# mazpie/genrl

Measured on AMD Instinct MI355X. Metric: world-model+imag update steps/sec (B32xL32x64x64x3), higher is better.
Workload: dtype f32 (storage, accumulation, every non-GEMM kernel and the fp32-MFMA GEMMs; the forward / dgrad / weight-gradient products of the imagination rollout, of the Dense+LN+SiLU chains from 192 rows up and of the encoder / decoder convolutions take fp32 operands pre-split into two fp16 planes of the scaled

## Files before the change

genrl_amd/csrc/gemm_planes.hip:

```cpp
#include "common.h"
#include "genrl_hip.h"
#include <type_traits>

typedef __bf16 bf16x8_t __attribute__((ext_vector_type(8)));
typedef _Float16 f16x8_t __attribute__((ext_vector_type(8)));
typedef unsigned u32x4 __attribute__((ext_vector_type(4)));

namespace {

struct PlaneSeg {
  const u16* a; long a_ld, a_plane;
  const u16* b; long b_ld, b_plane;
  int k;
  const float* a_inv; const float* b_inv;
};

struct SampleEpi {
  const float* q;
  long ldq;
  float* sample; long lds;
  u16* sp; long sld, splane; float* sinv;
  float a;
};

struct ConvGather {
  int H, W, C, k, Ho, Wo, K;
  int s;
  int sHo, sWo, sCo;
};

__device__ __host__ __forceinline__ long ln_slab(int tn) { return (long)(tn - 1) * 65536; }
struct LnEpi {
  const float* gamma; const float* beta;
  float eps; int act;
  float* y; long ldy;
  u16* yp; long yld, yplane; float* yinv;
  float* mean; float* rstd;
  float* part;
  unsigned* sync;
};

struct PairSel {
  const u16* b; long b_ld, b_plane; const float* b_inv;
  float* C; long ldc; int N, accumulate;
  int tn0, nx;
};

__device__ __forceinline__ float pow2_ratio(float a, float b) {
  const int ea = (int)((__builtin_bit_cast(unsigned, a) >> 23) & 255u), eb = (int)((__builtin_bit_cast(unsigned, b) >> 23) & 255u);
  const int e = min(max(ea - eb + 127, 1), 254);
  return __builtin_bit_cast(float, (unsigned)e << 23);
}
__device__ __forceinline__ bool zero_row_inv(float inv) { return __builtin_bit_cast(unsigned, inv) == (4u << 23); }

__device__ __forceinline__ void glds16(const void* g, unsigned lds_byte_addr) {
  __builtin_amdgcn_global_load_lds((const __attribute__((address_space(1))) void*)g,
                                   (__attribute__((address_space(3))) void*)(uintptr_t)lds_byte_addr, 16, 0, 0);
}

template <int N> __device__ __forceinline__ void wait_vm() { asm volatile("s_waitcnt vmcnt(%0)" ::"i"(N) : "memory"); }

template <int TM, int TN, int BK, int NACC, int FMT, int NS, bool FOLD, bool CONV, int PF, bool LNE, bool IS_PAIR>
__device__ __forceinline__ void gemm_planes_body(PlaneSeg s0, PlaneSeg s1, float* __restrict__ C, long ldc,
                                                 const float* __restrict__ bias, int M, int N, int accumulate,
                                                 int tiles_m, int tiles_n, int xcd_m, SampleEpi smp, ConvGather cg, LnEpi ln, PairSel pr) {
  static_assert(!LNE || (TM * TN == 1 && FMT == 1 && !CONV && PF == 0), "LayerNorm epilogue: 64x64 h2 tile");
  static_assert(!IS_PAIR || (TM * TN == 1 && FMT == 1 && !CONV && PF == 0 && !LNE), "pair of products: 64x64 h2 tile");
  constexpr int BM = 64 * TM, BN = 64 * TN;
  static_assert(!(FMT == 1 && FOLD) || (BM == 64 && BN == 64), "segment fold: 64x64 h2 tile");
  constexpr int NPL = FMT ? 2 : 3, NPROD = FMT ? 3 : 6;
  constexpr int ROWB = BK * 2;
  constexpr int CPR = ROWB / 16;
  constexpr int RPC = 1024 / ROWB;
  constexpr int A_BYTES = NPL * BM * ROWB, B_BYTES = NPL * BN * ROWB, STAGE = A_BYTES + B_BYTES;
  constexpr int APIECES = A_BYTES / 1024, BPIECES = B_BYTES / 1024;
  static_assert(APIECES % 2 == 0 && BPIECES % 2 == 0, "pieces split over two waves per operand");
  constexpr int NPA = APIECES / 2, NPB = BPIECES / 2;
  constexpr int NPMAX = NPA > NPB ? NPA : NPB;
  constexpr int KS = BK / 16;
  static_assert(PF == 0 || (BK == 64 && !CONV), "prefetch: 128-byte tile rows, plain operands");
  constexpr int NPF = PF ? TM : 0;
  constexpr int EPI = FMT == 1 ? 4 * (BM + 2 * BN) : 0, EPI_AT = NS * STAGE + (PF ? 1024 : 0);
  constexpr int LN_AT = EPI_AT + EPI, LN_G = LN_AT, LN_B = LN_AT + 4096, LN_R = LN_AT + 8192, LN_U = LN_AT + 9216, LN_T = LN_AT + 9472, LN_BYTES = LNE ? 9728 : 0;
  __shared__ __attribute__((aligned(1024))) unsigned char lds[EPI_AT + EPI + LN_BYTES];
// ... 1276 lines not shown
};
struct SplitBatch {
  int n;
  int blk0[33];
  SplitEntry e[32];
};
__device__ __forceinline__ int batch_entry(const SplitBatch& b, int blk) {
  int i = 0;
  while (i + 1 < b.n && blk >= b.blk0[i + 1]) ++i;
  return i;
}
__global__ __launch_bounds__(256) void split_h2_rows_batch_kernel(SplitBatch b) {
  const int i = batch_entry(b, blockIdx.x);
  const SplitEntry& e = b.e[i];
  const int row = (blockIdx.x - b.blk0[i]) * 4 + (threadIdx.x >> 6), lane = threadIdx.x & 63;
  if (row >= e.R) return;
  const float* xr = e.src + (long)row * e.ldx;
  float m = 0.f;
  for (int c = lane; c < e.Cn; c += 64) m = fmaxf(m, fabsf(xr[c]));
  const float iv = h2_inv_of(wave_max(m)), sc = h2_scale_of(iv);
  if (lane == 0) e.inv[row] = iv;
  u16* o = e.out + (long)row * e.ld_out;
  for (int c = 2 * lane; c < e.ld_out; c += 128) {
    unsigned h, l;
    h2_split2(c < e.Cn ? xr[c] * sc : 0.f, c + 1 < e.Cn ? xr[c + 1] * sc : 0.f, h, l);
    *reinterpret_cast<unsigned*>(o + c) = h;
    *reinterpret_cast<unsigned*>(o + e.plane + c) = l;
  }
}
__global__ __launch_bounds__(256) void h2_colmax_batch_kernel(SplitBatch b) {
  __shared__ float part[8][32];
  const int i = batch_entry(b, blockIdx.x);
  const SplitEntry& e = b.e[i];
  const int tx = threadIdx.x & 31, ty = threadIdx.x >> 5;
  const int c = (blockIdx.x - b.blk0[i]) * 32 + tx;
  float m = 0.f;
  if (c < e.Cn) {
    int r = ty;
    for (; r + 56 < e.R; r += 64) {
      float v[8];
#pragma unroll
      for (int u = 0; u < 8; ++u) v[u] = e.src[(long)(r + 8 * u) * e.ldx + c];
#pragma unroll
      for (int u = 0; u < 8; ++u) m = fmaxf(m, fabsf(v[u]));
    }
    for (; r < e.R; r += 8) m = fmaxf(m, fabsf(e.src[(long)r * e.ldx + c]));
  }
  part[ty][tx] = m;
  __syncthreads();
  if (ty == 0 && c < e.Cn) {
#pragma unroll
    for (int k = 1; k < 8; ++k) m = fmaxf(m, part[k][tx]);
    e.inv[c] = h2_inv_of(m);
  }
}
__global__ __launch_bounds__(256) void split_h2_t_batch_kernel(SplitBatch b) {
  __shared__ float tile[32][33];
  const int i = batch_entry(b, blockIdx.x);
  const SplitEntry& e = b.e[i];
  const int tiles_x = (int)((e.ld_out + 31) / 32);
  const int t = blockIdx.x - b.blk0[i];
  const int tx = threadIdx.x & 31, ty = threadIdx.x >> 5;
  const int ro = (t / tiles_x) * 32, co = (t % tiles_x) * 32;
#pragma unroll
  for (int k = 0; k < 4; ++k) {
    const int a = ty + 8 * k;
    const int r = co + a, c = ro + tx;
    tile[tx][a] = (r < e.R && c < e.Cn) ? e.src[(long)r * e.ldx + c] : 0.f;
  }
  __syncthreads();
#pragma unroll
  for (int k = 0; k < 4; ++k) {
    const int a = ty + 8 * k;
    const int r = ro + a, c = co + tx;
    if (r < e.Cn && c < e.ld_out) {
      unsigned h, l;
      h2_split2(c < e.R ? tile[a][tx] * h2_scale_of(e.inv[r]) : 0.f, 0.f, h, l);
      u16* o = e.out + (long)r * e.ld_out + c;
      o[0] = (u16)(h & 0xFFFFu); o[e.plane] = (u16)(l & 0xFFFFu);
    }
  }
}

static inline void log_launch(const char* family, long M, long N, long K, double bytes) { genrl_log_launch(family, M, N, K, bytes); }
static inline double kk_bytes(long M, long N, long K) { return 4.0 * ((double)M * K + (double)N * K + (double)M * N); }
static bool use_wide(int N) {
  static const int mode = getenv("GENRL_HL_WIDE") ? atoi(getenv("GENRL_HL_WIDE")) : 1;
  if (mode == 0) return false;
  const int c128 = cdiv(N, 128) * 128, c192 = cdiv(N, 192) * 192;
  return c192 < c128 || (mode == 2 && c192 == c128);
}
static bool use_tall96(int N, int K) {
  return N <= 96 && K >= 1024;
}
static bool hl_on() { static const bool on = !getenv("GENRL_PLANES_HL") || getenv("GENRL_PLANES_HL")[0] != '0'; return on; }
int g_planes_force_tile = 0;

}

unsigned g_planes_route = 0;
int g_planes_route_splits = 0;
static inline void route_reset() { g_planes_route = 0; g_planes_route_splits = 0; }
static inline void route(unsigned bit) { g_planes_route |= bit; }

extern "C" {

void genrl_log_launch(const char* family, long M, long N, long K, double operand_bytes) {
  static FILE* f = getenv("GENRL_GEMM_LOG") ? fopen(getenv("GENRL_GEMM_LOG"), "w") : nullptr;
  if (f) { fprintf(f, "%s %ld %ld %ld %.0f\n", family, M, N, K, operand_bytes); fflush(f); }
}

int genrl_planes_force_tile(int t) { const int p = g_planes_force_tile; g_planes_force_tile = t; return p; }
long genrl_planes_last_route(void) { return (long)g_planes_route | ((long)g_planes_route_splits << 32); }

int genrl_split_x3(const float* x, long ldx, int R, int Cn, uint16_t* out, long ld_out, long plane, int transpose,
                   void* stream) {
  GENRL_ENTER();
  const int Ro = transpose ? Cn : R, Co = transpose ? R : Cn;
  if (R <= 0 || Cn <= 0 || ld_out < Co) return GENRL_EINVAL;
  dim3 grid(cdiv(ld_out, 32), cdiv(Ro, 32));
  split_x3_kernel<<<grid, 256, 0, (hipStream_t)stream>>>(x, ldx, R, Cn, out, ld_out, plane, transpose);
  GENRL_CHECK_LAUNCH();
  return GENRL_OK;
}

static int xcd_split(int tm, int tn) {
  int best = 0; double bs = 1e30;
  for (int xm = 1; xm <= 8; xm *= 2) {
    const int xn = 8 / xm;
    if (tm % xm || tn % xn) continue;
    const double sm = (double)tm / xm, sn = (double)tn / xn, sc = sm + sn;
    if (sc < bs) { bs = sc; best = xm; }
  }
  return best;
}

int genrl_gemm_x3(const uint16_t* a0, long a0_ld, long a0_plane, const uint16_t* b0, long b0_ld, long b0_plane, int k0,
                  const uint16_t* a1, long a1_ld, long a1_plane, const uint16_t* b1, long b1_ld, long b1_plane, int k1,
                  float* C, long ldc, const float* bias, int M, int N, int accumulate, void* stream) {
  GENRL_ENTER();
  route_reset();
  if (M <= 0 || N <= 0 || k0 <= 0 || (k0 & 63) || (k1 & 63) || k1 < 0) return GENRL_EINVAL;
  if ((a0_ld & 7) || (b0_ld & 7) || (k1 && ((a1_ld & 7) || (b1_ld & 7)))) return GENRL_EINVAL;
  PlaneSeg s0{a0, a0_ld, a0_plane, b0, b0_ld, b0_plane, k0, nullptr, nullptr}, s1{a1, a1_ld, a1_plane, b1, b1_ld, b1_plane, k1, nullptr, nullptr};
  const long t64 = (long)cdiv(M, 64) * cdiv(N, 64);
  const bool big = g_planes_force_tile ? g_planes_force_tile == 2 : t64 >= 2048;
  if (big) {
    const int tm = cdiv(M, 128), tn = cdiv(N, 128);
    log_launch("x3/128", M, N, k0 + k1, 6.0 * ((double)M + N) * (k0 + k1) + 4.0 * M * N);
    route(GENRL_ROUTE_X3_128);
    gemm_planes_kernel<2, 2, 32, 1, 0, 3><<<tm * tn, 256, 0, (hipStream_t)stream>>>(s0, s1, C, ldc, bias, M, N, accumulate, tm, tn,
                                                                                xcd_split(tm, tn), SampleEpi{}, ConvGather{}, LnEpi{});
  } else {
    const int tm = cdiv(M, 64), tn = cdiv(N, 64);
    log_launch("x3/64", M, N, k0 + k1, 6.0 * ((double)M + N) * (k0 + k1) + 4.0 * M * N);
    route(GENRL_ROUTE_X3_64);
    gemm_planes_kernel<1, 1, 64, 3, 0, 3><<<tm * tn, 256, 0, (hipStream_t)stream>>>(s0, s1, C, ldc, bias, M, N, accumulate, tm, tn,
                                                                                xcd_split(tm, tn), SampleEpi{}, ConvGather{}, LnEpi{});
  }
  GENRL_CHECK_LAUNCH();
  return GENRL_OK;
}

int genrl_split_h2(const float* x, long ldx, int R, int Cn, uint16_t* out, long ld_out, long plane, float* inv, int transpose,
                   void* stream) {
  GENRL_ENTER();
  const int Co = transpose ? R : Cn;
  if (R <= 0 || Cn <= 0 || ld_out < Co || !inv || (ld_out & 63)) return GENRL_EINVAL;
  if (!transpose) {
    split_h2_rows_kernel<<<cdiv(R, 4), 256, 0, (hipStream_t)stream>>>(x, ldx, R, Cn, out, ld_out, plane, inv);
  } else {
    h2_colmax_kernel<<<cdiv(Cn, 32), 256, 0, (hipStream_t)stream>>>(x, ldx, R, Cn, inv);
    GENRL_CHECK_LAUNCH();
    dim3 grid(cdiv(ld_out, 32), cdiv(Cn, 32));
    split_h2_t_kernel<<<grid, 256, 0, (hipStream_t)stream>>>(x, ldx, R, Cn, out, ld_out, plane, inv);
  }
  GENRL_CHECK_LAUNCH();
  return GENRL_OK;
}

int genrl_split_h2_batch(const genrl_split_desc* d, int n, void* stream) {
  GENRL_ENTER();
  if (n < 0 || (n && !d)) return GENRL_EINVAL;
  for (int i = 0; i < n; ++i) {
    const int Co = d[i].transpose ? d[i].R : d[i].Cn;
    if (d[i].R <= 0 || d[i].Cn <= 0 || d[i].ld_out < Co || !d[i].inv || (d[i].ld_out & 63)) return GENRL_EINVAL;
  }
  hipStream_t s = (hipStream_t)stream;
  for (int pass = 0; pass < 2; ++pass) {
    int i = 0;
    while (i < n) {
      SplitBatch rows{}, cols{}, tiles{};
      int nb = 0;
      for (; i < n && nb < 32; ++i) {
        if ((d[i].transpose != 0) != (pass == 1)) continue;
        const SplitEntry e{d[i].src, d[i].ldx, d[i].R, d[i].Cn, d[i].out, d[i].ld_out, d[i].plane, d[i].inv};
        rows.e[nb] = cols.e[nb] = tiles.e[nb] = e;
        rows.blk0[nb + 1] = rows.blk0[nb] + cdiv(e.R, 4);
        cols.blk0[nb + 1] = cols.blk0[nb] + cdiv(e.Cn, 32);
        tiles.blk0[nb + 1] = tiles.blk0[nb] + cdiv(e.ld_out, 32) * cdiv(e.Cn, 32);
        ++nb;
      }
      if (!nb) continue;
      rows.n = cols.n = tiles.n = nb;
      if (pass == 0) {
        split_h2_rows_batch_kernel<<<rows.blk0[nb], 256, 0, s>>>(rows);
      } else {
        h2_colmax_batch_kernel<<<cols.blk0[nb], 256, 0, s>>>(cols);
        split_h2_t_batch_kernel<<<tiles.blk0[nb], 256, 0, s>>>(tiles);
      }
      GENRL_CHECK_LAUNCH();
    }
  }
  return GENRL_OK;
}

struct H2Route { bool big, two; };
static H2Route h2_route(int M, int N, int K, bool sample) {
  static const char* two_env = getenv("GENRL_PLANES_2PER");
  const long t64 = (long)cdiv(M, 64) * cdiv(N, 64);
  H2Route r;
  r.big = sample ? false : (g_planes_force_tile ? g_planes_force_tile == 2 : t64 >= 2048);
  r.two = !sample && (two_env ? two_env[0] == '1' : (t64 > 256 && K <= 1536));
  return r;
}

static int gemm_h2_impl(const uint16_t* a0, long a0_ld, long a0_plane, const float* a0_inv, const uint16_t* b0, long b0_ld, long b0_plane,
                        const float* b0_inv, int k0, const uint16_t* a1, long a1_ld, long a1_plane, const float* a1_inv,
                        const uint16_t* b1, long b1_ld, long b1_plane, const float* b1_inv, int k1,
                        float* C, long ldc, const float* bias, int M, int N, int accumulate, void* stream, const SampleEpi& smp) {
  GENRL_ENTER();
  if (M <= 0 || N <= 0 || k0 <= 0 || (k0 & 63) || (k1 & 63) || k1 < 0) return GENRL_EINVAL;
  if ((a0_ld & 7) || (b0_ld & 7) || (k1 && ((a1_ld & 7) || (b1_ld & 7)))) return GENRL_EINVAL;
  PlaneSeg s0{a0, a0_ld, a0_plane, b0, b0_ld, b0_plane, k0, a0_inv, b0_inv}, s1{a1, a1_ld, a1_plane, b1, b1_ld, b1_plane, k1, a1_inv, b1_inv};
  const H2Route rt = h2_route(M, N, k0 + k1, smp.q != nullptr);
  const bool big = rt.big;
  if (big && !g_planes_force_tile) {
    const int tm = cdiv(M, 128), tn = cdiv(N, 128), total = tm * tn, r = total % 256;
    if (total > 256 && r && r <= 128 && r % tn == 0 && (M & 127) == 0) {
      const int M1 = (tm - r / tn) * 128, M2 = M - M1;
      int rc = gemm_h2_impl(a0, a0_ld, a0_plane, a0_inv, b0, b0_ld, b0_plane, b0_inv, k0, a1, a1_ld, a1_plane, a1_inv, b1, b1_ld, b1_plane,
                            b1_inv, k1, C, ldc, bias, M1, N, accumulate, stream, smp);
      if (rc != GENRL_OK) return rc;
      return gemm_h2_impl(a0 + (long)M1 * a0_ld, a0_ld, a0_plane, a0_inv ? a0_inv + M1 : nullptr, b0, b0_ld, b0_plane, b0_inv, k0,
                          a1 ? a1 + (long)M1 * a1_ld : nullptr, a1_ld, a1_plane, a1_inv ? a1_inv + M1 : nullptr, b1, b1_ld, b1_plane, b1_inv, k1,
                          C + (long)M1 * ldc, ldc, bias, M2, N, accumulate, stream, smp);
    }
  }
  if (big) {
    const int tm = cdiv(M, 128), tn = cdiv(N, 128);
    const PlaneSeg none{nullptr, 0, 0, nullptr, 0, 0, 0, nullptr, nullptr};
    for (int seg = 0; seg < (k1 ? 2 : 1); ++seg) {
      const PlaneSeg& sg = seg ? s1 : s0;
      const float* bs = seg ? nullptr : bias;
      const int acc = seg ? 1 : accumulate;
      log_launch("h2/128", M, N, sg.k, kk_bytes(M, N, sg.k));
      route(!hl_on() ? GENRL_ROUTE_128_PLAIN : use_wide(N) ? GENRL_ROUTE_128_HLW : GENRL_ROUTE_128_HL);
      if (hl_on() && use_wide(N)) {
        const int tw = cdiv(N, 192);
        gemm_planes_hlw_kernel<false, 3><<<tm * tw, 256, 0, (hipStream_t)stream>>>(sg, C, ldc, bs, M, N, acc, tm, tw, xcd_split(tm, tw), ConvGather{});
      } else if (hl_on()) {
        gemm_planes_hl_kernel<false><<<tm * tn, 256, 0, (hipStream_t)stream>>>(sg, C, ldc, bs, M, N, acc, tm, tn, xcd_split(tm, tn) | (1 << 8), ConvGather{});
      } else
        gemm_planes_kernel<2, 2, 64, 2, 1, 2, false><<<tm * tn, 256, 0, (hipStream_t)stream>>>(sg, none, C, ldc, bs, M, N, acc, tm, tn,
                                                                                           xcd_split(tm, tn), SampleEpi{}, ConvGather{}, LnEpi{});
      GENRL_CHECK_LAUNCH();
    }
  } else {
    const int tm = cdiv(M, 64), tn = cdiv(N, 64);
    log_launch("h2/64", M, N, k0 + k1, kk_bytes(M, N, k0 + k1));
#define L64(NS_) gemm_planes_kernel<1, 1, 64, 3, 1, NS_, true><<<tm * tn, 256, 0, (hipStream_t)stream>>>( \
    s0, s1, C, ldc, bias, M, N, accumulate, tm, tn, xcd_split(tm, tn), smp, ConvGather{}, LnEpi{})
    const bool two = rt.two;
    route(smp.q ? GENRL_ROUTE_64_SAMPLE : (two ? GENRL_ROUTE_64_NS2 : GENRL_ROUTE_64_NS3));
    if (two) L64(2);
    else L64(3);
#undef L64
  }
  GENRL_CHECK_LAUNCH();
  return GENRL_OK;
}

int genrl_gemm_h2_conv(const uint16_t* img, long ld_img, long plane_img, const float* img_inv, int Nimg, int H, int W, int Cc, int k,
                       const uint16_t* b, long b_ld, long b_plane, const float* b_inv, float* C, long ldc, const float* bias, int N,
                       int accumulate, void* stream) {
  GENRL_ENTER();
  route_reset();
  const int Ho = (H - k) / 2 + 1, Wo = (W - k) / 2 + 1, K = k * k * Cc;
  const long Ml = (long)Nimg * Ho * Wo;
  if (Nimg <= 0 || Ho <= 0 || Wo <= 0 || N <= 0 || (Cc & 7) || Cc < 48 || ld_img < Cc || (ld_img & 7) || (b_ld & 63) || b_ld < K || b_ld >= K + 64 || K < 64 ||
      !img_inv || !b_inv || Ml > 0x7fffffffL)
    return GENRL_EINVAL;
  if ((((long)Nimg * H * W * ld_img + plane_img) * 2) >= 0xffffffffL) return GENRL_EINVAL;
  const int M = (int)Ml;
  PlaneSeg s0{img, ld_img, plane_img, b, b_ld, b_plane, (int)b_ld, img_inv, b_inv};
  const PlaneSeg none{nullptr, 0, 0, nullptr, 0, 0, 0, nullptr, nullptr};
  const bool wide = hl_on() && use_wide(N);
// ... 133 lines not shown
```

genrl_amd/planes.py:

```python
import os
import weakref
import torch
from ._lib import lib, check, GenrlHipError, struct

ENABLED = os.environ.get('GENRL_PLANES', '1') != '0'
_amp_saved = None
gemm_profile = None


from .streams import raw_current_stream as _stream
from .streams import timed_start, timed_end


def r64(k):
    return (k + 63) // 64 * 64


class Planes:
    __slots__ = ('t', 'inv', 'rows', 'cols', 'ld', 'plane', 'uniform')

    def __init__(self, rows, cols, dev, zero=True):
        self.rows, self.cols, self.ld = rows, cols, r64(cols)
        self.uniform = False
        mk = torch.zeros if (self.ld != cols and zero) else torch.empty
        self.t = mk(2, rows, self.ld, dtype=torch.int16, device=dev)
        self.inv = torch.empty(rows, device=dev)
        self.plane = rows * self.ld

    def ptr(self, row0=0):
        return self.t.data_ptr() + 2 * row0 * self.ld

    def inv_ptr(self, row0=0):
        return self.inv.data_ptr() + 4 * row0

    def float(self):
        f = lambda t: t.view(torch.float16).double()
        return ((f(self.t[0]) + f(self.t[1]) / 2048.0) * self.inv.double()[:, None])[:, :self.cols].float()


def split(x2d, transpose=False, out=None, row0=0):
    assert x2d.dim() == 2 and x2d.dtype == torch.float32 and (x2d.shape[1] == 1 or x2d.stride(1) == 1)
    R, C = x2d.shape
    Ro, Co = (C, R) if transpose else (R, C)
    if out is None:
        out = Planes(Ro, Co, x2d.device)
    assert out.cols == Co and row0 + Ro <= out.rows
    check(lib().genrl_split_h2(x2d.data_ptr(), x2d.stride(0), R, C, out.ptr(row0), out.ld, out.plane, out.inv_ptr(row0),
                               int(transpose), _stream()), 'split_h2')
    return out


_epoch = 0
_wcache = {}


_dcache = {}


def derived(W, tag, build, extra=None):
    if not isinstance(W, torch.nn.Parameter):
        return build()
    key, st = (id(W), tag), _stream()
    ent = _dcache.get(key)
    ver = (W._version, extra)
    fresh = ent is not None and ent[0] == _epoch and ent[2] == W.data_ptr() and ent[3]() is W and ent[5] == ver
    if not fresh or ent[4] != st:
        if ent is None:
            weakref.finalize(W, _dcache.pop, key, None)
        ent = _dcache[key] = [_epoch, build(), W.data_ptr(), weakref.ref(W), st, ver]
    return ent[1]


def invalidate(params=None):
    global _epoch
    if params is None:
        _epoch += 1
        return
    ids = {id(q) for q in params}
    for key, ent in _wcache.items():
        if key[0] in ids:
            ent[0] = -1
    for key, ent in _dcache.items():
        if key[0] in ids:
            ent[0] = -1


def _split_entries(stale, stream):
    if not stale:
        return
    arr = (struct('genrl_split_desc') * len(stale))()
    for d, ((_, transpose, c0, c1), ent) in zip(arr, stale):
        W, P = ent[3](), ent[1]
        d.src, d.ldx, d.R, d.Cn = W.data_ptr() + 4 * c0 * W.stride(1), W.stride(0), W.shape[0], c1 - c0
        d.out, d.ld_out, d.plane, d.inv, d.transpose = P.ptr(0), P.ld, P.plane, P.inv_ptr(0), int(transpose)
    check(lib().genrl_split_h2_batch(arr, len(stale), stream), 'split_h2_batch')
    for _, ent in stale:
        ent[0], ent[2] = _epoch, ent[3]().data_ptr()


def _refresh_stale(stream):
    _split_entries([(key, ent) for key, ent in _wcache.items() if ent[0] != _epoch and ent[4] == stream and ent[3]() is not None], stream)


def refresh(params):
    ids = {id(q) for q in params}
    _split_entries([(key, ent) for key, ent in _wcache.items() if key[0] in ids and ent[3]() is not None], _stream())


def weight(W, transpose=False, c0=0, c1=None):
    c1 = W.shape[1] if c1 is None else c1
    if not isinstance(W, torch.nn.Parameter):
        return split(W.detach()[:, c0:c1], transpose)
    key = (id(W), transpose, c0, c1)
    ent = _wcache.get(key)
    st = _stream()
    if ent is None or ent[2] != W.data_ptr() or ent[3]() is not W:
        rows, cols = (c1 - c0, W.shape[0]) if transpose else (W.shape[0], c1 - c0)
        assert W.dim() == 2 and W.stride(1) == 1
        if ent is None:
            weakref.finalize(W, _wcache.pop, key, None)
        ent = _wcache[key] = [-1, Planes(rows, cols, W.device), W.data_ptr(), weakref.ref(W), st]
    ent[4] = st
    if ent[0] != _epoch:
        _refresh_stale(st)
    return ent[1]


def gemm(A, B, C, ldc, bias, M, N, accumulate=False, a_row0=0, A1=None, B1=None, a1_row0=0, c_off=0, b_row0=0, b1_row0=0):
    assert A.ld == B.ld and a_row0 + M <= A.rows and b_row0 + N <= B.rows, (A.ld, B.ld, A.rows, B.rows, M, N)
    e0 = timed_start(gemm_profile)
    k1 = 0
    a1 = b1 = (None, 0, 0, None)
    if A1 is not None:
        assert A1.ld == B1.ld and a1_row0 + M <= A1.rows and b1_row0 + N <= B1.rows
        k1 = A1.ld
        a1, b1 = (A1.ptr(a1_row0), A1.ld, A1.plane, A1.inv_ptr(a1_row0)), (B1.ptr(b1_row0), B1.ld, B1.plane, B1.inv_ptr(b1_row0))
    check(lib().genrl_gemm_h2(A.ptr(a_row0), A.ld, A.plane, A.inv_ptr(a_row0), B.ptr(b_row0), B.ld, B.plane, B.inv_ptr(b_row0),
                              A.ld, *a1, *b1, k1, C.data_ptr() + 4 * c_off, ldc, bias.data_ptr() if bias is not None else None,
                              M, N, int(accumulate), _stream()), 'gemm_h2')
    timed_end(gemm_profile, e0, M, N, A.cols + (A1.cols if A1 is not None else 0), 'kk/h2/pipe4')


def gemm_pair(A, B0, C0, ldc0, N0, acc0, B1, C1, ldc1, N1, acc1, M):
    assert A.ld == B0.ld == B1.ld and M <= A.rows and N0 <= B0.rows and N1 <= B1.rows
    e0 = timed_start(gemm_profile)
    rc = lib().genrl_gemm_h2_pair(A.ptr(0), A.ld, A.plane, A.inv_ptr(0), A.ld,
                                  B0.ptr(0), B0.ld, B0.plane, B0.inv_ptr(0), C0.data_ptr(), ldc0, N0, int(acc0),
                                  B1.ptr(0), B1.ld, B1.plane, B1.inv_ptr(0), C1.data_ptr(), ldc1, N1, int(acc1), M, _stream())
    if rc == 1:
        gemm(A, B0, C0, ldc0, None, M, N0, accumulate=acc0)
        gemm(A, B1, C1, ldc1, None, M, N1, accumulate=acc1)
        return
    check(rc, 'gemm_h2_pair')
    timed_end(gemm_profile, e0, M, N0 + N1, A.cols, 'kk/h2/pipe4')


LN_FUSED = os.environ.get('GENRL_GEMM_LN', '1') != '0'
_ln_ws = {}


def _ln_workspace(dev):
    d = torch.device(dev).index
    d = torch.cuda.current_device() if d is None else d
    ws = _ln_ws.get(d)
    if ws is None:
        if torch.cuda.is_current_stream_capturing():
            return None
        L = lib()
        ws = _ln_ws[d] = (torch.zeros(L.genrl_gemm_h2_ln_sync_words(), dtype=torch.int32, device=f'cuda:{d}'),
                          torch.zeros(L.genrl_gemm_h2_ln_part_floats(1024, 1024) + 4, device=f'cuda:{d}'))
    return ws


def ln_fused_here(dev=None):
    if not (LN_FUSED and ENABLED):
        return False
    from . import streams
    return not streams.on_side_stream() and _ln_workspace(dev if dev is not None else torch.cuda.current_device()) is not None


def gemm_ln_ok(M, N, dev=None):
    return LN_FUSED and ENABLED and lib().genrl_gemm_h2_ln_ok(M, N) == 1 and ln_fused_here(dev)


def gemm_ln(A, B, C, bias, M, N, gamma, beta, eps, out_p, out_row0, y=None, mean=None, rstd=None, act=True, a_row0=0, A1=None, B1=None,
            a1_row0=0, c_off=0, y_off=0, m_off=0):
    assert A.ld == B.ld and a_row0 + M <= A.rows and N <= B.rows and out_p.cols == N and out_row0 + M <= out_p.rows
    k1 = 0
    a1 = b1 = (None, 0, 0, None)
# ... 72 lines not shown
```

include/genrl_hip.h:

```cpp
#ifndef GENRL_HIP_H
#define GENRL_HIP_H
#include <stdint.h>
#ifdef __cplusplus
extern "C" {
#endif

long genrl_sgemm_ws_floats(int M, int N, int K);
int genrl_set_gemm_precision(int mode);
int genrl_sgemm_last_pipe(void);
int genrl_gemm_precision(void);
int genrl_sgemm(const float* A, long a_rs, long a_ks, const float* B, long b_rs, long b_ks, float* C, long ldc,
                const float* bias, int M, int N, int K, int accumulate, float* ws, long ws_floats, void* stream);

int genrl_sgemm_conv(const float* A, long a_rs, long a_ks, const float* B, long b_rs, long b_ks, float* C, long ldc,
                     const float* bias, int M, int N, int K, int accumulate, float* ws, long ws_floats, int which,
                     int img_h, int img_w, int img_c, int ksize, void* stream);

int genrl_split_h2(const float* x, long ldx, int R, int Cn, uint16_t* out, long ld_out, long plane, float* inv, int transpose,
                   void* stream);
int genrl_gemm_h2(const uint16_t* a0, long a0_ld, long a0_plane, const float* a0_inv, const uint16_t* b0, long b0_ld, long b0_plane,
                  const float* b0_inv, int k0, const uint16_t* a1, long a1_ld, long a1_plane, const float* a1_inv,
                  const uint16_t* b1, long b1_ld, long b1_plane, const float* b1_inv, int k1,
                  float* C, long ldc, const float* bias, int M, int N, int accumulate, void* stream);
int genrl_gemm_h2_pair(const uint16_t* a, long a_ld, long a_plane, const float* a_inv, int k,
// ... 52 lines not shown
typedef struct { const uint16_t* p; long ld, plane; const float* inv; } genrl_planes_ref;
typedef struct {
  int H, N, S, K, D, A, AP, U, L;
  float unimix, min_std, max_std;
  float* stoch; float* deter; float* logit; float* action; float* raws;
  const float* eps; const float* q;
  genrl_planes_ref stoch_p, deter_p, act_p, x_p, o_p;
  float* x_pre; float* x; float* g_pre; float* o_pre; float* o;
  float* xm; float* xr; float* gm; float* gr; float* om; float* orr;
  genrl_planes_ref w_in_s, w_in_a, w_g_x, w_g_h, w_out, w_dist;
  const float* in_b; const float* in_g; const float* in_be; float in_eps;
  const float* gru_g; const float* gru_be;
  const float* out_b; const float* out_g; const float* out_be; float out_eps;
  const float* dist_b;
  genrl_planes_ref pw0s, pw0d;
  genrl_planes_ref pw[8]; const float* pb[8]; const float* pg[8]; const float* pbe[8]; float peps[8]; int pU[8];
  float* ppre[8]; float* py[8]; float* pmean[8]; float* prstd[8]; genrl_planes_ref pyp[8];
  const float* head_w; const float* head_b;
  float* ln_part; unsigned* ln_sync;
} genrl_rollout;
int genrl_imagine_seq_fwd(const genrl_rollout* r, void* stream);
typedef struct {
  int H, N, S, K, D, A, AP, U;
  float unimix, min_std, max_std;
  const float* logit; const float* deter; const float* raws; const float* eps; const float* x_pre; const float* g_pre; const float* o_pre;
  const float* xm; const float* xr; const float* gm; const float* gr; const float* om; const float* orr;
  float* ds; float* dd; const float* dl_in; const float* dact_all; float* d_raw;
  float* dlg; float* dov; float* do_pre; float* dg_pre; float* dx; float* dx_pre; float* dha; float* dhb;
  genrl_planes_ref dlg_p, dop_p, dg_p, dxp_p;
  genrl_planes_ref wt_dist, wt_out, wt_g_x, wt_g_h, wt_in_s;
  const float* waT;
  const float* out_g; const float* out_be; const float* gru_g; const float* gru_be; const float* in_g; const float* in_be;
  float* dx_pre_all;
} genrl_rollout_bwd;
int genrl_imagine_seq_bwd(const genrl_rollout_bwd* r, void* stream);
typedef struct {
  int H, N, S, K, D, A, AP, U, L;
  float unimix, min_std, max_std;
  float* stoch; float* deter; float* logit; float* action; float* raws; const float* eps; const float* q;
  float* x_pre; float* x; float* g_pre; float* o_pre; float* o;
  float* xm; float* xr; float* gm; float* gr; float* om; float* orr;
  const float* ws_in; const float* wa; const float* gru_w; const float* out_w; const float* dist_w;
  const float* in_b; const float* in_g; const float* in_be; float in_eps; const float* gru_g; const float* gru_be;
  const float* out_b; const float* out_g; const float* out_be; float out_eps; const float* dist_b;
  const float* pw[8]; const float* pb[8]; const float* pg[8]; const float* pbe[8]; float peps[8]; int pU[8];
  float* ppre[8]; float* py[8]; float* pmean[8]; float* prstd[8];
  const float* head_w; const float* head_b;
  float* ws; long ws_floats;
  float* ds; float* dd; const float* dl_in; const float* dact_all; float* d_raw;
  float* dlg; float* dov; float* do_pre; float* dg_pre; float* dx; float* dx_pre; float* dha; float* dhb; const float* waT;
} genrl_rollout_f32;
int genrl_imagine_seq_f32_fwd(const genrl_rollout_f32* r, void* stream);
int genrl_imagine_seq_f32_bwd(const genrl_rollout_f32* r, void* stream);

typedef struct {
  int T, B, S, K, D, U;
  float unimix, in_eps, out_eps;
  const float* w_in_s; long ld_in_s; const float* w_g; long ld_g; const float* w_o; long ld_o; const float* w_d;
  const float* in_g; const float* in_be; const float* gru_g; const float* gru_be; const float* out_g; const float* out_be;
  const float* dist_b; const float* mask; const float* q;
  const float* out_b; int opre_acc;
  int* idx; const float* w_in_sT; int fuse_sample;
  float* sm; float* xpre; float* xh; float* gpre; float* deter; float* opre; float* o; float* plog; float* pst;
  float* xm; float* xr; float* gm; float* gr; float* om; float* orr;
  float* ws; long ws_floats;
  const float* d_pst; float* dlg; float* dd; float* dov; float* dopre; float* dgpre; float* dxh; float* dxpre;
  float* dsa; float* dsb; float* dhd_a; float* dhd_b; float* dgamma; float* dbeta; float* gws; int direct;
} genrl_observe;
int genrl_observe_seq_fwd(const genrl_observe* r, void* stream);
int genrl_observe_seq_bwd(const genrl_observe* r, int* final_buf, void* stream);
long genrl_gemm_h2_tn_ws_bytes(int NI, int NJ, int M);
int genrl_gemm_h2_tn(const uint16_t* a, long a_ld, long a_plane, const float* a_inv, const uint16_t* b, long b_ld, long b_plane,
                     const float* b_inv, float* C, long ldc, int NI, int NJ, int M, int accumulate, void* ws, long ws_bytes,
                     void* stream);
int genrl_gemm_h2_tn_conv(const uint16_t* a, long a_ld, long a_plane, const float* a_inv, const uint16_t* img, long ld_img,
                          long plane_img, const float* img_inv, const unsigned* rowoff, int W, int Cc, int k, float* C, long ldc,
                          int NI, int M, int accumulate, void* ws, long ws_bytes, void* stream);
typedef struct {
  const float* src; long ldx; int R, Cn;
  uint16_t* out; long ld_out, plane; float* inv;
  int transpose;
} genrl_split_desc;
int genrl_split_h2_batch(const genrl_split_desc* descs, int n, void* stream);
int genrl_split_x3(const float* x, long ldx, int R, int Cn, uint16_t* out, long ld_out, long plane, int transpose,
                   void* stream);
int genrl_gemm_x3(const uint16_t* a0, long a0_ld, long a0_plane, const uint16_t* b0, long b0_ld, long b0_plane, int k0,
                  const uint16_t* a1, long a1_ld, long a1_plane, const uint16_t* b1, long b1_ld, long b1_plane, int k1,
                  float* C, long ldc, const float* bias, int M, int N, int accumulate, void* stream);
int genrl_planes_force_tile(int t);
long genrl_planes_last_route(void);
#define GENRL_ROUTE_64_NS3        0x1u
#define GENRL_ROUTE_64_NS2        0x2u
#define GENRL_ROUTE_64_SAMPLE     0x4u
#define GENRL_ROUTE_64_LN         0x8u
#define GENRL_ROUTE_128_PLAIN     0x10u
#define GENRL_ROUTE_128_HL        0x20u
#define GENRL_ROUTE_128_HLW       0x40u
#define GENRL_ROUTE_CONV_PLAIN    0x80u
#define GENRL_ROUTE_CONV_HL       0x100u
#define GENRL_ROUTE_CONV_HLW      0x200u
#define GENRL_ROUTE_CONV_TALL96   0x400u
#define GENRL_ROUTE_SUBPIXEL_HL   0x800u
#define GENRL_ROUTE_SUBPIXEL_HLW  0x1000u
#define GENRL_ROUTE_X3_64         0x2000u
#define GENRL_ROUTE_X3_128        0x4000u
#define GENRL_ROUTE_TN            0x8000u
#define GENRL_ROUTE_TN_CONV       0x10000u

int genrl_ln_act_fwd_h2(const float* x, long ldx, const float* gamma, const float* beta, float* y, long ldy, float* mean,
                        float* rstd, int M, int N, float eps, int act, uint16_t* yp, long ldp, long plane, float* inv,
                        void* stream);
typedef struct {
  const float* part; float* out0; float* out1; float* out2;
  int nchunk, N, np, accumulate;
} genrl_reduce_desc;
int genrl_ln_bwd_parts(int M, int N);
int genrl_reduce_params_batch(const genrl_reduce_desc* descs, int n, void* stream);
int genrl_ln_act_bwd_h2(const float* dy, long lddy, const float* x, long ldx, const float* gamma, const float* beta,
                        const float* mean, const float* rstd, float* dx, long lddx, float* dgamma, float* dbeta,
                        float* dcolsum, float* ws, int M, int N, int act, int accumulate_params, uint16_t* dxp, long ldp,
                        long plane, float* inv, void* stream);
int genrl_gru_gates_fwd_h2(const float* pre, const float* h, long ldh, const float* gamma, const float* beta,
                           float* hout, long ldo, float* hout2, const float* hout2_scale, float* mean, float* rstd,
                           int R, int D, float eps, uint16_t* hp, long ldp, long plane, float* inv, void* stream);
int genrl_gru_gates_bwd_h2(const float* dhout, long lddo, const float* dhout2, const float* dhout2_scale,
                           const float* pre, const float* h, long ldh, const float* gamma, const float* beta,
                           const float* mean, const float* rstd, float* dpre, float* dh, long lddh, float* dgamma,
                           float* dbeta, float* ws, int R, int D, int accumulate_params, const float* dhout2_parts,
                           int nparts, long part_stride, uint16_t* dprep, long ldp, long plane, float* inv, void* stream);
int genrl_actor_head_fwd_h2(const float* raw, const float* eps, float* action, float* mean, float* std, long R, int A,
                            float min_std, float max_std, long ld_action, uint16_t* ap, long ldp, long plane, float* inv,
                            void* stream);
int genrl_onehot_fwd_h2(const float* logits, const float* q, float* sample, float* probs, long G, int K, float unimix,
                        uint16_t* sp, int rowlen, long ldp, long plane, float* inv, void* stream);
int genrl_onehot_bwd_planes_only_ok(int K, int rowlen);
int genrl_onehot_bwd_h2(const float* logits, const float* gsample, float* dlogits, long G, int K, float unimix,
                        int accumulate, uint16_t* dp, int rowlen, long ldp, long plane, float* inv, void* stream);

int genrl_sgemm_skinny_parts(const float* A, long a_rs, const float* B, long b_rs, long b_ks, float* P, long ldp,
                             long part_stride, int M, int N, int K, int nparts, void* stream);

int genrl_ln_act_fwd(const float* x, long ldx, const float* gamma, const float* beta, float* y, long ldy, float* mean,
                     float* rstd, int M, int N, float eps, int act, void* stream);
long genrl_ln_ws_floats(int M, int N);
int genrl_ln_act_bwd(const float* dy, long lddy, const float* x, long ldx, const float* gamma, const float* beta,
                     const float* mean, const float* rstd, float* dx, long lddx, float* dgamma, float* dbeta,
                     float* dcolsum, float* ws, int M, int N, int act, int accumulate_params, void* stream);
long genrl_colsum_ws_floats(int M, int N);
int genrl_colsum(const float* x, long ldx, float* out, float* ws, int M, int N, int accumulate, void* stream);

int genrl_gru_gates_fwd(const float* pre, const float* h, long ldh, const float* gamma, const float* beta,
                        float* hout, long ldo, float* hout2, const float* hout2_scale, float* mean, float* rstd,
                        int R, int D, float eps, void* stream);
int genrl_gru_gates_fwd_ld2(const float* pre, const float* h, long ldh, const float* gamma, const float* beta,
                            float* hout, long ldo, float* hout2, long ldo2, const float* hout2_scale, float* mean, float* rstd,
                            int R, int D, float eps, void* stream);
long genrl_gru_ws_floats(int R, int D);
int genrl_gru_gates_bwd(const float* dhout, long lddo, const float* dhout2, const float* dhout2_scale,
                        const float* pre, const float* h, long ldh, const float* gamma, const float* beta,
                        const float* mean, const float* rstd, float* dpre, float* dh, long lddh, float* dgamma,
                        float* dbeta, float* ws, int R, int D, int accumulate_params, const float* dhout2_parts,
                        int nparts, long part_stride, void* stream);
int genrl_gru_gates_bwd_ldp(const float* dhout, long lddo, const float* dhout2, const float* dhout2_scale,
                            const float* pre, const float* h, long ldh, const float* gamma, const float* beta,
                            const float* mean, const float* rstd, float* dpre, float* dh, long lddh, float* dgamma,
                            float* dbeta, float* ws, int R, int D, int accumulate_params, const float* dhout2_parts,
// ... 150 lines not shown
```

Before: 47.82.

## Add unified weight-plane split kernel with fused column max and transpose

Result: no change. 47.88, median of 5 (+0.1%).

```diff
diff --git a/genrl_amd/csrc/gemm_planes.hip b/genrl_amd/csrc/gemm_planes.hip
--- a/genrl_amd/csrc/gemm_planes.hip
+++ b/genrl_amd/csrc/gemm_planes.hip
@@ -1,5 +1,6 @@
 #include "common.h"
 #include "genrl_hip.h"
+#include "weight_planes.h"
 #include <type_traits>
 
 typedef __bf16 bf16x8_t __attribute__((ext_vector_type(8)));
@@ -1442,6 +1443,125 @@
   }
 }
 
+using wplanes::Entry;
+template <int KIND>
+__device__ __forceinline__ float wp_x(const Entry& e, int r, int c) {
+  if constexpr (KIND == GENRL_WP_ROWS) {
+    return e.src[(long)r * e.ldx + c];
+  } else if constexpr (KIND == GENRL_WP_PERM) {
+    const int q = c / e.p0, b = c - q * e.p0;
+    return e.src[((long)r * e.p0 + b) * e.p1 + q];
+  } else {
+    const int Ci = e.p0, Co = e.p1, k = e.p2, T = (k + 1) >> 1;
+    const int cls = r / Co, co = r - cls * Co, tap = c / Ci, ci = c - tap * Ci, u = tap / T, v = tap - u * T;
+    const int kh = (cls >> 1) + 2 * (T - 1 - u), kw = (cls & 1) + 2 * (T - 1 - v);
+    return (kh < k && kw < k) ? e.src[ci * e.ldx + co * e.s_co + (kh * k + kw) * e.s_tap] : 0.f;
+  }
+}
+template <int KIND>
+__device__ __forceinline__ void wp_rows(const Entry& e, int row, int lane) {
+  float m = 0.f;
+  for (int c = lane; c < e.Cn; c += 64) m = fmaxf(m, fabsf(wp_x<KIND>(e, row, c)));
+  const float iv = h2_inv_of(wave_max(m)), sc = h2_scale_of(iv);
+  if (lane == 0) e.inv[row] = iv;
+  u16* o = e.out + (long)row * e.ld_out;
+  for (int c = 2 * lane; c < e.ld_out; c += 128) {
+    const float v0 = c < e.Cn ? wp_x<KIND>(e, row, c) : 0.f, v1 = c + 1 < e.Cn ? wp_x<KIND>(e, row, c + 1) : 0.f;
+    unsigned h, l;
+    h2_split2(v0 * sc, v1 * sc, h, l);
+    *reinterpret_cast<unsigned*>(o + c) = h;
+    *reinterpret_cast<unsigned*>(o + e.plane + c) = l;
+  }
+}
+template <int KIND>
+__device__ __forceinline__ void wp_cols(const Entry& e, int stripe, int chunk, float (*tile)[32][33], float (*part)[32]) {
+  const int tx = threadIdx.x & 31, ty = threadIdx.x >> 5;
+  const int c0 = stripe * 32, c = c0 + tx;
+  const int R = e.R, Cn = e.Cn;
+  float m = 0.f;
+  if (c < Cn) {
+    int r = ty;
+    for (; r + 120 < R; r += 128) {
+      float v[16];
+#pragma unroll
+      for (int u = 0; u < 16; ++u) v[u] = wp_x<KIND>(e, r + 8 * u, c);
+#pragma unroll
+      for (int u = 0; u < 16; ++u) m = fmaxf(m, fabsf(v[u]));
+    }
+    for (; r < R; r += 8) m = fmaxf(m, fabsf(wp_x<KIND>(e, r, c)));
+  }
+  part[ty][tx] = m;
+  __syncthreads();
+  if (ty == 0) {
+#pragma unroll
+    for (int k = 1; k < 8; ++k) m = fmaxf(m, part[k][tx]);
+    const float iv = h2_inv_of(m);
+    if (c < Cn && chunk == 0) e.inv[c] = iv;
+    part[0][tx] = h2_scale_of(iv);
+  }
+  const int ntiles = (int)(e.ld_out >> 5);
+  const int t0 = chunk * wplanes::T_TILES, t1 = min(t0 + wplanes::T_TILES, ntiles);
+  const int px = threadIdx.x & 15, py = threadIdx.x >> 4;
+  float v[4];
+#pragma unroll
+  for (int k = 0; k < 4; ++k) {
+    const int r = t0 * 32 + ty + 8 * k;
+    v[k] = (r < R && c < Cn) ? wp_x<KIND>(e, r, c) : 0.f;
+  }
+  for (int t = t0; t < t1; ++t) {
+    float (*tl)[33] = tile[(t - t0) & 1];
+#pragma unroll
+    for (int k = 0; k < 4; ++k) tl[tx][ty + 8 * k] = v[k];
+    if (t + 1 < t1) {
+#pragma unroll
+      for (int k = 0; k < 4; ++k) {
+        const int r = (t + 1) * 32 + ty + 8 * k;
+        v[k] = (r < R && c < Cn) ? wp_x<KIND>(e, r, c) : 0.f;
+      }
+    }
+    __syncthreads();
+    const int col = t * 32 + 2 * px;
+#pragma unroll
+    for (int j = 0; j < 2; ++j) {
+      const int a = py + 16 * j, orow = c0 + a;
+      if (orow < Cn) {
+        const float sc = part[0][a];
+        unsigned h, l;
+        h2_split2(col < R ? tl[a][2 * px] * sc : 0.f, col + 1 < R ? tl[a][2 * px + 1] * sc : 0.f, h, l);
+        u16* o = e.out + (long)orow * e.ld_out + col;
+        *reinterpret_cast<unsigned*>(o) = h;
+        *reinterpret_cast<unsigned*>(o + e.plane) = l;
+      }
+    }
+  }
+}
+__global__ __launch_bounds__(256) void weight_planes_batch_kernel(wplanes::Batch b) {
+  __shared__ float tile[2][32][33];
+  __shared__ float part[8][32];
+  int i = 0;
+  while (i + 1 < b.n && (int)blockIdx.x >= b.blk0[i + 1]) ++i;
+  const Entry& e = b.e[i];
+  const int blk = blockIdx.x - b.blk0[i];
+  if (e.kind == GENRL_WP_ROWS_T || e.kind == GENRL_WP_PERM_T) {
+    const int nch = (int)((e.ld_out / 32 + wplanes::T_TILES - 1) / wplanes::T_TILES);
+    if (e.kind == GENRL_WP_ROWS_T) wp_cols<GENRL_WP_ROWS>(e, blk / nch, blk % nch, tile, part);
+    else wp_cols<GENRL_WP_PERM>(e, blk / nch, blk % nch, tile, part);
+    return;
+  }
+  const int row = blk * 4 + (threadIdx.x >> 6), lane = threadIdx.x & 63;
+  if (row >= e.R) return;
+  switch (e.kind) {
+    case GENRL_WP_ROWS: wp_rows<GENRL_WP_ROWS>(e, row, lane); break;
+    case GENRL_WP_PERM: wp_rows<GENRL_WP_PERM>(e, row, lane); break;
+    case GENRL_WP_SUBPIXEL:
+      wp_rows<GENRL_WP_SUBPIXEL>(e, row, lane);
+      if (e.bias && lane == 0) e.f32[row] = e.bias[row % e.p1];
+      break;
+    default:
+      for (int c = lane; c < e.Cn; c += 64) e.f32[(long)row * e.Cn + c] = wp_x<GENRL_WP_PERM>(e, row, c);
+  }
+}
+
 static inline void log_launch(const char* family, long M, long N, long K, double bytes) { genrl_log_launch(family, M, N, K, bytes); }
 static inline double kk_bytes(long M, long N, long K) { return 4.0 * ((double)M * K + (double)N * K + (double)M * N); }
 static bool use_wide(int N) {
@@ -1573,6 +1693,15 @@
     }
   }
   return GENRL_OK;
+}
+
+int genrl_weight_planes_batch(const genrl_wplane_desc* d, int n, void* stream) {
+  GENRL_ENTER();
+  return wplanes::for_each_chunk(d, n, [&](const wplanes::Batch& b, int nblk) {
+    weight_planes_batch_kernel<<<nblk, 256, 0, (hipStream_t)stream>>>(b);
+    GENRL_CHECK_LAUNCH();
+    return (int)GENRL_OK;
+  });
 }
 
 struct H2Route { bool big, two; };
diff --git a/genrl_amd/csrc/weight_planes.h b/genrl_amd/csrc/weight_planes.h
--- /dev/null
+++ b/genrl_amd/csrc/weight_planes.h
@@ -0,0 +1,67 @@
+#pragma once
+#include <cstdint>
+#include "genrl_hip.h"
+#ifndef GENRL_OK
+#define GENRL_OK 0
+#define GENRL_EINVAL 1
+#endif
+
+namespace wplanes {
+
+constexpr int CHUNK = 32;
+constexpr int T_TILES = 16;
+
+struct Entry {
+  const float* src; const float* bias;
+  uint16_t* out; float* inv; float* f32;
+  long ldx, s_co, s_tap, ld_out, plane;
+  int kind, R, Cn, p0, p1, p2;
+};
+struct Batch {
+  int n;
+  int blk0[CHUNK + 1];
+  Entry e[CHUNK];
+};
+
+static inline bool transposed(int kind) { return kind == GENRL_WP_ROWS_T || kind == GENRL_WP_PERM_T; }
+
+static inline bool valid(const genrl_wplane_desc& d) {
+  if (d.kind < GENRL_WP_ROWS || d.kind > GENRL_WP_PERM_COPY || d.R <= 0 || d.Cn <= 0 || !d.src) return false;
+  if (d.kind == GENRL_WP_PERM || d.kind == GENRL_WP_PERM_T || d.kind == GENRL_WP_PERM_COPY) {
+    if (d.p0 <= 0 || d.p1 <= 0 || (long)d.p0 * d.p1 != d.Cn) return false;
+  }
+  if (d.kind == GENRL_WP_PERM_COPY) return d.f32 != nullptr;
+  if (d.kind == GENRL_WP_SUBPIXEL) {
+    const long T = (d.p2 + 1) / 2;
+    if (d.p0 <= 0 || d.p1 <= 0 || d.p2 < 1 || 4L * d.p1 != d.R || T * T * d.p0 != d.Cn || (d.bias != nullptr) != (d.f32 != nullptr)) return false;
+  }
+  const int Co = transposed(d.kind) ? d.R : d.Cn;
+  return d.out && d.inv && d.ld_out >= Co && !(d.ld_out & 63);
+}
+
+static inline int cdiv_(long a, long b) { return (int)((a + b - 1) / b); }
+static inline int t_chunks(long ld_out) { return cdiv_(ld_out / 32, T_TILES); }
+static inline int blocks(const genrl_wplane_desc& d) {
+  return transposed(d.kind) ? cdiv_(d.Cn, 32) * t_chunks(d.ld_out) : cdiv_(d.R, 4);
+}
+
+template <typename Launch>
+int for_each_chunk(const genrl_wplane_desc* d, int n, Launch&& launch) {
+  if (n < 0 || (n && !d)) return GENRL_EINVAL;
+  for (int i = 0; i < n; ++i)
+    if (!valid(d[i])) return GENRL_EINVAL;
+  for (int i0 = 0; i0 < n; i0 += CHUNK) {
+    Batch b{};
+    b.n = n - i0 < CHUNK ? n - i0 : CHUNK;
+    for (int j = 0; j < b.n; ++j) {
+      const genrl_wplane_desc& s = d[i0 + j];
+      b.e[j] = Entry{s.src, s.bias, s.out, s.inv, s.f32, s.ldx, s.s_co, s.s_tap, s.ld_out, s.plane, s.kind, s.R, s.Cn, s.p0, s.p1, s.p2};
+      b.blk0[j + 1] = b.blk0[j] + blocks(s);
+    }
+    const int rc = launch(b, b.blk0[b.n]);
+    if (rc != GENRL_OK) return rc;
+  }
+  return GENRL_OK;
+}
+
+}
diff --git a/genrl_amd/planes.py b/genrl_amd/planes.py
--- a/genrl_amd/planes.py
+++ b/genrl_amd/planes.py
@@ -85,26 +85,38 @@
             ent[0] = -1
 
 
+WP_ROWS, WP_ROWS_T = 0, 1
+
+
 def _split_entries(stale, stream):
     if not stale:
         return
-    arr = (struct('genrl_split_desc') * len(stale))()
-    for d, ((_, transpose, c0, c1), ent) in zip(arr, stale):
-        W, P = ent[3](), ent[1]
-        d.src, d.ldx, d.R, d.Cn = W.data_ptr() + 4 * c0 * W.stride(1), W.stride(0), W.shape[0], c1 - c0
-        d.out, d.ld_out, d.plane, d.inv, d.transpose = P.ptr(0), P.ld, P.plane, P.inv_ptr(0), int(transpose)
-    check(lib().genrl_split_h2_batch(arr, len(stale), stream), 'split_h2_batch')
-    for _, ent in stale:
-        ent[0], ent[2] = _epoch, ent[3]().data_ptr()
+    arr = (struct('genrl_wplane_desc') * len(stale))()
+    for d, ((_, transpose, c0, c1), ent, W) in zip(arr, stale):
+        P = ent[1]
+        d.kind, d.src, d.ldx, d.R, d.Cn = (WP_ROWS_T if transpose else WP_ROWS), W.data_ptr() + 4 * c0 * W.stride(1), W.stride(0), W.shape[0], c1 - c0
+        d.out, d.ld_out, d.plane, d.inv = P.ptr(0), P.ld, P.plane, P.inv_ptr(0)
+    check(lib().genrl_weight_planes_batch(arr, len(stale), stream), 'weight_planes_batch')
+    for _, ent, W in stale:
+        ent[0], ent[2] = _epoch, W.data_ptr()
+
+
+def _alive(pick):
+    out = []
+    for key, ent in list(_wcache.items()):
+        W = ent[3]()
+        if W is not None and pick(key, ent):
+            out.append((key, ent, W))
+    return out
 
 
 def _refresh_stale(stream):
-    _split_entries([(key, ent) for key, ent in _wcache.items() if ent[0] != _epoch and ent[4] == stream and ent[3]() is not None], stream)
+    _split_entries(_alive(lambda key, ent: ent[0] != _epoch and ent[4] == stream), stream)
 
 
 def refresh(params):
     ids = {id(q) for q in params}
-    _split_entries([(key, ent) for key, ent in _wcache.items() if key[0] in ids and ent[3]() is not None], _stream())
+    _split_entries(_alive(lambda key, ent: key[0] in ids), _stream())
 
 
 def weight(W, transpose=False, c0=0, c1=None):
diff --git a/include/genrl_hip.h b/include/genrl_hip.h
--- a/include/genrl_hip.h
+++ b/include/genrl_hip.h
@@ -158,6 +158,15 @@
   int transpose;
 } genrl_split_desc;
 int genrl_split_h2_batch(const genrl_split_desc* descs, int n, void* stream);
+enum { GENRL_WP_ROWS = 0, GENRL_WP_ROWS_T = 1, GENRL_WP_PERM = 2, GENRL_WP_PERM_T = 3, GENRL_WP_SUBPIXEL = 4, GENRL_WP_PERM_COPY = 5 };
+typedef struct {
+  const float* src; const float* bias;
+  long ldx, s_co, s_tap;
+  int kind, R, Cn, p0, p1, p2;
+  uint16_t* out; long ld_out, plane; float* inv;
+  float* f32;
+} genrl_wplane_desc;
+int genrl_weight_planes_batch(const genrl_wplane_desc* descs, int n, void* stream);
 int genrl_split_x3(const float* x, long ldx, int R, int Cn, uint16_t* out, long ld_out, long plane, int transpose,
                    void* stream);
 int genrl_gemm_x3(const uint16_t* a0, long a0_ld, long a0_plane, const uint16_t* b0, long b0_ld, long b0_plane, int k0,
```
